# david-cortes/recometrics

Hardware: AMD Instinct MI355X
Metric: users/sec evaluated (all metrics, K=10) (higher is better)
Workload: dtype f32

## Files before the change

### recometrics_amd/csrc/rm_lib.hip

```cpp
#include <hip/hip_runtime.h>

#include <algorithm>
#include <array>
#include <cmath>
#include <cstdio>
#include <cstring>
#include <cstdlib>
#include <type_traits>
#include <atomic>
#include <chrono>
#include <condition_variable>
#include <csignal>
#include <functional>
#include <limits>
#include <map>
#include <memory>
#include <mutex>
#include <string>
#include <thread>
#include <vector>

#include "../../include/recometrics_hip.h"
#include "rm_device.hpp"
#include "rm_prep.hpp"
#include "rm_launch.hpp"
#include "rm_finalize.hpp"
#include "rm_noise.hpp"
#include "rm_scores.hpp"
#include "rm_rowtopk.hpp"

namespace {

using namespace rm;

thread_local std::string g_err;
struct RmError { int code; std::string msg; };

#define HIP_CHECK(expr)                                                                                   \
    do {                                                                                                  \
        hipError_t e_ = (expr);                                                                           \
        if (e_ != hipSuccess)                                                                             \
            throw RmError{e_ == hipErrorOutOfMemory ? RM_ERR_NOMEM : RM_ERR_HIP,                          \
                          std::string(#expr) + ": " + hipGetErrorString(e_)};                             \
    } while (0)

struct Switches {
    bool no_train_bits, no_spec, no_side, ext_topk, no_test_mask, hbm_lists, nsub2, no_pending, no_pos_beside, no_seed, rank_generic,
         no_fused_auc, no_defer_auc, noise_sequential, one_context, noise_per_batch, host_trace, no_pos_flat, no_row_topk, no_split_cache;
    long long free_mb, stream_budget_mb, noise_budget_mb, lane_cap_min, lane_min_k, lane_cap_set, sample_seed, split_cache_mb;
    unsigned long long epoch = 0;
    double batch_users;
    std::string splits;
    static bool on(const char *name) { return getenv(name) != nullptr; }
    static long long num(const char *name) { const char *e = getenv(name); return e ? atoll(e) : -1; }
    void load()
    {
        no_train_bits = on("RM_DEBUG_NO_TRAIN_BITS"); no_spec = on("RM_DEBUG_NO_SPEC"); no_side = on("RM_DEBUG_NO_SIDE");
        ext_topk = on("RM_DEBUG_EXT_TOPK"); no_test_mask = on("RM_DEBUG_NO_TEST_MASK");
        hbm_lists = on("RM_DEBUG_HBM_LISTS"); nsub2 = on("RM_DEBUG_NSUB2"); no_pending = on("RM_DEBUG_NO_PENDING");
        no_pos_beside = on("RM_DEBUG_NO_POS_BESIDE"); no_seed = on("RM_DEBUG_NO_SEED");
        rank_generic = on("RM_DEBUG_RANK_GENERIC"); no_fused_auc = on("RM_DEBUG_NO_FUSED_AUC");
        no_defer_auc = on("RM_DEBUG_NO_DEFER_AUC"); noise_sequential = on("RM_DEBUG_NOISE_SEQUENTIAL");
        one_context = on("RM_DEBUG_ONE_CONTEXT"); noise_per_batch = on("RM_DEBUG_NOISE_PER_BATCH"); host_trace = on("RM_HOST_TRACE");
        no_pos_flat = on("RM_DEBUG_NO_POS_FLAT");
        no_row_topk = on("RM_DEBUG_NO_ROW_TOPK");
        free_mb = num("RM_DEBUG_FREE_MB"); stream_budget_mb = num("RM_STREAM_BUDGET_MB");
        noise_budget_mb = num("RM_NOISE_BUDGET_MB");
        lane_min_k = num("RM_DEBUG_LANE_MIN_K");
        lane_cap_set = num("RM_DEBUG_LANE_CAP");
        sample_seed = num("RM_DEBUG_SAMPLE_SEED");
        lane_cap_min = num("RM_DEBUG_LANE_CAP_MIN");
        no_split_cache = on("RM_DEBUG_NO_SPLIT_CACHE");
        split_cache_mb = num("RM_SPLIT_CACHE_MB");
        epoch++;
        const char *b = getenv("RM_BATCH_USERS"); batch_users = b ? atof(b) : 0.0;
        const char *s = getenv("RM_DEBUG_SPLITS"); splits = s ? s : "";
    }
    Switches() { load(); }
};
Switches g_sw;

std::atomic<long long> g_ws_bytes{0};
inline long long debug_free_cap()
{
    return g_sw.free_mb >= 0 ? (g_sw.free_mb << 20) : -1;
}

struct RunTrace {
    std::mutex mu; std::vector<std::pair<const char *, double>> pts; std::chrono::steady_clock::time_point t0 = std::chrono::steady_clock::now();
    void point(const char *what) { std::lock_guard<std::mutex> lk(mu); if (pts.size() > 4096) pts.clear(); pts.emplace_back(what, std::chrono::duration<double, std::milli>(std::chrono::steady_clock::now() - t0).count()); }
};
RunTrace g_run_trace;
#define RM_TRACE_POINT(what) do { if (g_sw.host_trace) g_run_trace.point(what); } while (0)

std::atomic<unsigned long long> g_ws_stamp{1};
// ... 52 lines not shown
constexpr long long SPLIT_CACHE_DEFAULT_MB = 1024;
struct SplitKey {
    const void *arr[SPLIT_ARRAYS]; long long words[SPLIT_ARRAYS], nnz_train, nnz_test;
    int m, n, k, K, elem, req, min_items_pool, min_pos_test, heavy_npos, ng;
    int cold, cumulative, want_lane, ext_topk, allow_stream, force_stream, dense_ok, flat_early, csr_checked, rank_out;
    unsigned long long switches;
};
struct SplitCache {
    static constexpr const char *copy_names[SPLIT_ARRAYS] = {"split_train_p", "split_train_i", "split_test_p", "split_test_i", "split_test_v"};
    bool valid = false; SplitKey key{}; Plan hp{}; bool check_nan = false, dense_masked = false;
    std::vector<std::pair<std::string, unsigned long long>> stamps;
    void invalidate() { valid = false; }
    void keep(const Workspace &ws, const char *name) { stamps.emplace_back(name, ws.peek(name).stamp); }
    bool holds(const Workspace &ws, const SplitKey &k) const
    {
        if (!valid || std::memcmp(&key, &k, sizeof(SplitKey)) != 0) return false;
        for (const auto &s : stamps) if (s.second == 0 || ws.peek(s.first.c_str()).stamp != s.second) return false;
        return true;
    }
    const void *copy(const Workspace &ws, int i) const { return ws.peek(copy_names[i]).ptr; }
};
enum SideMark { SIDE_FORK, SIDE_JOIN, SIDE_PLAN_FORK, SIDE_CHECKS_DONE, SIDE_ROWS_AND_PACKS, SIDE_ROWS_FOR_POS, SIDE_TOP_VALUES,
                SIDE_SWEEP_FORK, SIDE_SWEEP_DEEP_DONE, SIDE_MERGED, SIDE_VERDICT, SIDE_SPLIT_KEPT, SIDE_MARKS };
enum PosMark { POS_PLAN_FORK, POS_MAXIMA_DONE, POS_SCORES_AFTER_COPY, POS_SCORES_DONE, POS_TABLES_INIT, POS_STREAMED_PLACED, POS_MARKS };
enum PassEvent { EV_START, EV_PREP_END , EV_SWEEP_END, EV_END, EV_COUNT };
struct NoiseWords {
    int first_early;
    int first_final;
    int sequential;
    int range_early;
    int batch_flagged;
};
static_assert(sizeof(NoiseWords) <= 64, "the noise words share one 64-byte page-locked allocation");
struct Ctx {
    int device = 0, slot = 0;
    std::mutex mu;
    Workspace ws;
    hipEvent_t ev[EV_COUNT] = {nullptr, nullptr, nullptr, nullptr};
    bool ev_valid = false, ev_recorded = false;
    hipStream_t side_stream = nullptr; std::array<hipEvent_t, SIDE_MARKS> side_marks{};
    hipStream_t pos_stream = nullptr; std::array<hipEvent_t, POS_MARKS> pos_marks{};
    hipEvent_t done = nullptr;
    hipStream_t own_stream = nullptr;
    hipStream_t up_stream = nullptr;
    hipEvent_t up_ev[2] = {nullptr, nullptr};
    NoiseWords *noise_words = nullptr; hipEvent_t flags_ev = nullptr, pass_ev = nullptr;
    void need_noise_words()
    {
        if (noise_words) return;
        HIP_CHECK(hipHostMalloc((void **)&noise_words, 64, hipHostMallocDefault));
        HIP_CHECK(hipEventCreateWithFlags(&flags_ev, hipEventDisableTiming));
        HIP_CHECK(hipEventCreateWithFlags(&pass_ev, hipEventDisableTiming));
    }
    void *pinned = nullptr; size_t pinned_bytes = 0;
    void *pinned_get(size_t bytes)
    {
        if (pinned_bytes < bytes) {
            if (pinned) { (void)hipHostFree(pinned); pinned = nullptr; pinned_bytes = 0; }
            if (hipHostMalloc(&pinned, bytes + bytes / 8, hipHostMallocDefault) != hipSuccess) { pinned = nullptr; throw RmError{RM_ERR_NOMEM, "hipHostMalloc of the output staging buffer failed"}; }
            pinned_bytes = bytes + bytes / 8;
        }
        return pinned;
    }
    double timings[8] = {0, 0, 0, 0, 0, 0, 0, 0};
// ... 326 lines not shown
inline void launch_csr_checks(int m, int n, const int *train_p, const int *train_i, long long nnz_train, const int *test_p, const int *test_i, long long nnz_test,
                              Plan *plan, const unsigned char *, hipStream_t stream)
{
    hipLaunchKernelGGL(k_check_csr_ptr, dim3(cdiv(m, 256)), dim3(256), 0, stream, m, train_p, nnz_train, test_p, nnz_test, plan);
    launch_csr_index_checks(m, n, train_p, train_i, nnz_train, test_p, test_i, nnz_test, plan, stream);
}
template <class T>
void check_csr_now(const Call<T> &c, hipStream_t stream, Ctx &cx)
{
    Plan *plan = (Plan *)cx.ws.get("plan", sizeof(Plan));
    cx.split.invalidate();
    if (cx.ev_valid) HIP_CHECK(hipStreamWaitEvent(stream, cx.done, 0));
    HIP_CHECK(hipMemsetAsync(plan, 0, sizeof(Plan), stream));
    launch_csr_checks(c.m, c.n, c.train_p, c.train_i, c.nnz_train, c.test_p, c.test_i, c.nnz_test, plan, c.only_users, stream);
    Plan hp;
    HIP_CHECK(hipMemcpyAsync(&hp, plan, sizeof(Plan), hipMemcpyDeviceToHost, stream));
    HIP_CHECK(hipStreamSynchronize(stream));
    throw_csr_defects(hp, c, cx);
}

struct Beside {
    hipStream_t &st; hipEvent_t *const ev; const int n_ev; const hipStream_t call; const bool high_priority; bool enabled;
    long long handed = 0, joined = 0, at[SIDE_MARKS] = {};
    static_assert((int)POS_MARKS <= (int)SIDE_MARKS, "at[] holds the roles of either stream");
    Beside(hipStream_t &s, hipEvent_t *e, int n, hipStream_t call_, bool hp, bool on_) : st(s), ev(e), n_ev(n), call(call_), high_priority(hp), enabled(on_) {}
    ~Beside() { if (handed > joined && st) (void)hipStreamSynchronize(st); }
    hipStream_t get()
    {
        if (!st) {
            HIP_CHECK(create_stream(&st, high_priority));
            for (int i = 0; i < n_ev; i++) HIP_CHECK(hipEventCreateWithFlags(&ev[i], hipEventDisableTiming));
        }
        return st;
    }
    hipStream_t on() { if (!enabled) return call; handed++; return get(); }
    void cut(int role) { if (enabled) { get(); HIP_CHECK(hipEventRecord(ev[role], call)); } }
    hipStream_t behind(int role) { if (!enabled) return call; HIP_CHECK(hipStreamWaitEvent(st, ev[role], 0)); handed++; return st; }
    hipStream_t fork(int role) { cut(role); return behind(role); }
    void mark(int role) { if (enabled) { HIP_CHECK(hipEventRecord(ev[role], st)); at[role] = handed; } }
    void joined_at(int role) { joined = std::max(joined, at[role]); at[role] = 0; }
    void await(int role, hipStream_t into) { if (enabled) { HIP_CHECK(hipStreamWaitEvent(into, ev[role], 0)); if (into == call) joined_at(role); } }
    void join(int role) { mark(role); await(role, call); }
    bool marked(int role) const { return at[role] != 0; }
    void sync() { if (enabled && st) { HIP_CHECK(hipStreamSynchronize(st)); joined = handed; } }
    void host_wait(int role) { if (enabled) { HIP_CHECK(hipEventSynchronize(ev[role])); joined_at(role); } }
};

// ... 88 lines not shown

inline Geometry scores_geometry(const Plan &hp, int n, bool want_auc)
{
    Geometry g{};
    g.jmax = want_auc ? hp.jmax : 0;
    g.n_ublocks = (hp.n_groups + GROUPS_PER_BLOCK - 1) / GROUPS_PER_BLOCK;
    g.nsub = 2; g.tile_items = TILE_ITEMS; g.n_waves = 8;
    g.tiles_total = (n + TILE_ITEMS - 1) / TILE_ITEMS;
    g.n_splits = 1; g.part_splits = 1; g.n_part = 1;
    g.u_split = 0; g.j_shallow = -1;
    return g;
}

template <class T>
struct Pipeline {
    typedef Prec<T> P;
    typedef typename std::remove_pointer<decltype(typename P::Args{}.thr_shared)>::type ThrT;
    static constexpr int GU = P::GU;
    Call<T> c;
    hipStream_t stream; Ctx &cx; Workspace &ws;
    const int m, n, k, K;
    const bool use_side = !g_sw.no_side;
    Beside side, pos;
    int min_items_pool = 0, min_pos_test = 0, req = 0, NG = 0; bool want_auc = false;
    int *flags = nullptr, *user_nslots = nullptr, *uslot_base = nullptr, *heavy_users = nullptr; Plan *plan = nullptr;
    int *slot_user = nullptr, *slot_chunk = nullptr, *slot_index = nullptr, *gj = nullptr, *sc_user = nullptr, *sc_chunk = nullptr;
    long long *grow = nullptr; double *log2tab = nullptr;
    ClassifyArgs ca{};
    bool want_lane = false, ext_topk = false, items_known = false, dense_ok = false;
    bool row_topk = false;
    bool bits_early = false, bits_early_masked = false, masked_from_bits = false, flat_early = false;
    bool allow_reuse = true, reused = false, keepable = false; SplitKey split_key{};
    Plan hp{};
    int n_slots = 0, n_stream = 0, stream_slot0 = 0; bool check_nan = false;
    Geometry g{};
    FinalArgs<T, T> fa{};
    Entry<T> *merged = nullptr; long long *rank_sorted = nullptr;
    T *pos_score = nullptr; unsigned *hist = nullptr; int *pos_order = nullptr, *pos_item = nullptr;
    Entry<T> *pl = nullptr; PartialStat<T> *pst = nullptr;
    T *stream_scores = nullptr, *spos_score = nullptr; int *spos_item = nullptr; unsigned *shist = nullptr;
    long long stream_ld = 0;
    typename P::Args sa{};
    typename P::ListT *glists = nullptr; int *lane_cnt = nullptr; ThrT *thr_shared = nullptr;
    bool lane_lists = false;
    bool collect = false; CollectGeom collect_g{};

    Pipeline(const Call<T> &c_, hipStream_t s, Ctx &cx_)
        : c(c_), stream(s), cx(cx_), ws(cx_.ws), m(c_.m), n(c_.n), k(c_.k), K(c_.K),
          side(cx_.side_stream, cx_.side_marks.data(), SIDE_MARKS, s, cx_.high_priority, use_side),
          pos(cx_.pos_stream, cx_.pos_marks.data(), POS_MARKS, s, cx_.high_priority, use_side) {}

    void begin()
    {
        min_items_pool = std::max(std::max(c.min_items_pool, K), 2);
        min_pos_test = std::min(c.min_pos_test, 1);
        if (c.reco) { min_items_pool = 1; min_pos_test = 0; }
        for (int i = 0; i < 10; i++) if (c.out[i] && !c.reco) req |= (1 << i);
        want_auc = req & (RQ_ROC | RQ_PR);
        NG = c.scores ? 2 : P::supported_ng(k);
        if (NG < 0) throw RmError{RM_ERR_UNSUPPORTED, std::string(P::limit()) + " (got " + std::to_string(k) + ")"};
        if (!cx.ev_valid) {
            for (int i = 0; i < EV_COUNT; i++) HIP_CHECK(hipEventCreate(&cx.ev[i]));
            HIP_CHECK(hipEventCreateWithFlags(&cx.done, hipEventDisableTiming));
            cx.ev_valid = true;
        } else {
            HIP_CHECK(hipStreamWaitEvent(stream, cx.done, 0));
        }
        g_last_ctx = &cx;
        HIP_CHECK(hipEventRecord(cx.ev[EV_START], stream));
        RM_TRACE_POINT("run: start");
    }

    void plan_stage()
// ... 97 lines not shown
            side.mark(SIDE_CHECKS_DONE);
            if (!c.scores) hipLaunchKernelGGL(k_absmax<T>, dim3(512), dim3(256), 0, aux2, c.A, c.lda, (long long)m, k, &plan->amax_a, &plan->nonfinite);
            if (!items_known && !c.scores) hipLaunchKernelGGL(k_absmax<T>, dim3(1024), dim3(256), 0, aux2, c.B, c.ldb, (long long)n, k, &plan->amax_b, &plan->nonfinite_b);
            pos.mark(POS_MAXIMA_DONE);
            if (attempt == 0 && flat_early) hipLaunchKernelGGL(k_entry_users, dim3(cdiv(cdiv(m, WAVE) * WAVE, 256)), dim3(256), 0, pos.on(), m, c.test_p, ent_user, plan);
            if (attempt == 0 && std::is_same<T, float>::value && use_side && !c.ext_bits && dense_ok) {
                SweepArgs probe{};
                const bool guess = want_auc && !ext_topk && !g_sw.no_test_mask;
                (void)ws.get("train_bits", (size_t)m * (size_t)dense_row_words(n) * 4);
                if (!(c.same_train_rows && cx.dense.fits(ws, m, dense_row_words(n), guess))) {
                    set_train_bits(probe, cx, c, m, n, dense_ok, side.on(), guess, false, false, flat_early ? ent_masked : nullptr);
                    side.mark(SIDE_ROWS_AND_PACKS); side.mark(SIDE_ROWS_FOR_POS);
                    bits_early = true; bits_early_masked = guess; masked_from_bits = flat_early;
                }
            }
            side.await(SIDE_CHECKS_DONE, stream); pos.await(POS_MAXIMA_DONE, stream);
            HIP_CHECK(hipMemcpyAsync(cx.pinned_plan, plan, sizeof(Plan), hipMemcpyDeviceToHost, stream));
            if (attempt == 0 && flat_early) {
                const hipStream_t sc = pos.fork(POS_SCORES_AFTER_COPY);
                if (c.scores) {
                    hipLaunchKernelGGL(k_test_masked, dim3(cdiv(m, TM_USERS)), dim3(256), 0, sc, m, c.test_p, c.test_i, c.train_p, c.train_i, ent_user, ent_masked, plan);
                    hipLaunchKernelGGL(k_pos_scores_given<T>, dim3(cdiv(c.nnz_test, 256)), dim3(256), 0, sc, pf, c.S, c.lds, (const int *)ent_user, (const unsigned char *)ent_masked);
                } else {
                hipLaunchKernelGGL(k_pos_scores_flat<T>, dim3(cdiv(c.nnz_test, POSF_WAVES * WAVE)), dim3(POSF_WAVES * WAVE), 0, sc, pf, ent_user);
                if (masked_from_bits) side.await(SIDE_ROWS_FOR_POS, sc);
                else hipLaunchKernelGGL(k_test_masked, dim3(cdiv(m, TM_USERS)), dim3(256), 0, sc, m, c.test_p, c.test_i, c.train_p, c.train_i, ent_user, ent_masked, plan);
                hipLaunchKernelGGL(k_pos_apply_masked<T>, dim3(cdiv(c.nnz_test, 256)), dim3(256), 0, sc, pf, ent_masked);
                }
                pos.mark(POS_SCORES_DONE);
            }
            RM_TRACE_POINT("run: plan chain + side kernels enqueued");
            HIP_CHECK(hipStreamSynchronize(stream));
            RM_TRACE_POINT("run: plan read back");
            hp = *cx.pinned_plan;
            throw_csr_defects(hp, c, cx);
            if (ca.allow_stream && !ca.force_stream && hp.class_count[STREAM_CLASS] > stream_cap && attempt == 0) {
                ca.allow_stream = 0; ca.check_ptr = 0; keepable = false;
                side.sync(); pos.sync();
                continue;
            }
            break;
        }
        if (!reused) throw_csr_defects(hp, c, cx);
        n_slots = hp.n_slots;
        n_stream = (want_auc || ext_topk) ? hp.class_count[STREAM_CLASS] : 0;
        stream_slot0 = n_stream > 0 ? hp.class_offset[STREAM_CLASS] : n_slots;
        if (!reused) check_nan = scores_may_overflow();
// ... 12 lines not shown
    bool make_split_key(SplitKey &key) const
    {
        std::memset(&key, 0, sizeof(SplitKey));
        if (g_sw.no_split_cache || !use_side || c.reco || c.scores || c.noise || c.only_users || c.ext_bits || c.noise_E || c.noise_flag ||
            c.first_pass_flags || c.flag_snapshot || c.items_tag != 0 || !c.test_p || m <= 0) return false;
        const void *arr[SPLIT_ARRAYS] = {c.train_p, c.train_i, c.test_p, c.test_i, c.test_v};
        const long long words[SPLIT_ARRAYS] = {(long long)m + 1, std::max<long long>(c.nnz_train, 0), (long long)m + 1, std::max<long long>(c.nnz_test, 0),
                                               c.test_v ? std::max<long long>(c.nnz_test, 0) * (long long)(sizeof(T) / 4) : 0};
        long long total = 0;
        for (int i = 0; i < SPLIT_ARRAYS; i++) { key.arr[i] = arr[i]; key.words[i] = words[i]; total += words[i]; }
        if (total * 4 > ((g_sw.split_cache_mb >= 0 ? g_sw.split_cache_mb : SPLIT_CACHE_DEFAULT_MB) << 20)) return false;
        key.nnz_train = c.nnz_train; key.nnz_test = c.nnz_test;
        key.m = m; key.n = n; key.k = k; key.K = K; key.elem = (int)sizeof(T); key.req = req;
        key.min_items_pool = min_items_pool; key.min_pos_test = min_pos_test; key.heavy_npos = ca.heavy_npos; key.ng = NG;
        key.cold = c.cold; key.cumulative = c.cumulative; key.want_lane = want_lane; key.ext_topk = ext_topk;
        key.allow_stream = ca.allow_stream; key.force_stream = ca.force_stream; key.dense_ok = dense_ok; key.flat_early = flat_early;
        key.csr_checked = c.csr_checked; key.rank_out = (c.topk_idx ? 1 : 0) | (c.pos_rank ? 2 : 0) | (c.status ? 4 : 0);
        key.switches = g_sw.epoch;
        return true;
    }
    void plan_reused(const PosArgs<T> &pf, const int *ent_user, const unsigned char *ent_masked, const void *const theirs[SPLIT_ARRAYS])
    {
        const SplitCache &kept = cx.split;
        const size_t at = offsetof(Plan, split_differs);
        HIP_CHECK(hipMemsetAsync((char *)plan + at, 0, offsetof(Plan, csr_bad) - at, stream));
        const hipStream_t aux = side.fork(SIDE_PLAN_FORK);
        SplitSameArgs ss{};
        long long longest = 1;
        for (int i = 0; i < SPLIT_ARRAYS; i++) {
            ss.theirs[i] = (const unsigned *)theirs[i]; ss.ours[i] = (const unsigned *)kept.copy(ws, i); ss.words[i] = kept.key.words[i];
            longest = std::max(longest, ss.words[i]);
        }
        ss.plan = plan;
        const unsigned blocks = (unsigned)std::min<long long>(SPLIT_SAME_BLOCKS, cdiv(cdiv(longest, 4), SPLIT_SAME_THREADS));
        hipLaunchKernelGGL(k_split_same, dim3(blocks), dim3(SPLIT_SAME_THREADS), 0, aux, ss);
        hipLaunchKernelGGL(k_absmax<T>, dim3(512), dim3(256), 0, aux, c.A, c.lda, (long long)m, k, &plan->amax_a, &plan->nonfinite);
        hipLaunchKernelGGL(k_absmax<T>, dim3(1024), dim3(256), 0, aux, c.B, c.ldb, (long long)n, k, &plan->amax_b, &plan->nonfinite_b);
        HIP_CHECK(hipMemcpyAsync(cx.pinned_plan, plan, sizeof(Plan), hipMemcpyDeviceToHost, aux));
        side.mark(SIDE_VERDICT);
        if (flat_early) {
            const hipStream_t sc = pos.fork(POS_PLAN_FORK);
            hipLaunchKernelGGL(k_pos_scores_flat<T>, dim3(cdiv(c.nnz_test, POSF_WAVES * WAVE)), dim3(POSF_WAVES * WAVE), 0, sc, pf, ent_user);
            hipLaunchKernelGGL(k_pos_apply_masked<T>, dim3(cdiv(c.nnz_test, 256)), dim3(256), 0, sc, pf, ent_masked);
            pos.mark(POS_SCORES_DONE);
        }
        check_launch(hipGetLastError());
        hp = kept.hp; check_nan = kept.check_nan;
        bits_early = dense_ok; bits_early_masked = kept.dense_masked; masked_from_bits = true;
        RM_TRACE_POINT("run: kept split, comparison + positives enqueued");
    }
    bool verdict()
    {
        side.host_wait(SIDE_VERDICT);
        RM_TRACE_POINT("run: verdict read back");
        const Plan &rb = *cx.pinned_plan;
        hp.amax_a = rb.amax_a; hp.amax_b = rb.amax_b; hp.nonfinite = rb.nonfinite; hp.nonfinite_b = rb.nonfinite_b;
        if (!rb.split_differs && scores_may_overflow() == check_nan) { cx.split_reused = 1; return true; }
        side.sync(); pos.sync();
        HIP_CHECK(hipStreamSynchronize(stream));
        cx.split.invalidate(); cx.dense.invalidate(); cx.packed.invalidate();
        cx.split_reused = 0;
        return false;
    }
    void keep_split()
    {
        if (!keepable || reused) return;
        SplitCache &kept = cx.split;
        void *dst[SPLIT_ARRAYS] = {};
        try { for (int i = 0; i < SPLIT_ARRAYS; i++) if (split_key.words[i] > 0) dst[i] = ws.get(SplitCache::copy_names[i], (size_t)split_key.words[i] * 4); }
        catch (const RmError &) { keepable = false; return; }
        const hipStream_t st = side.on();
        for (int i = 0; i < SPLIT_ARRAYS; i++)
            if (dst[i]) HIP_CHECK(hipMemcpyAsync(dst[i], split_key.arr[i], (size_t)split_key.words[i] * 4, hipMemcpyDeviceToDevice, st));
        side.mark(SIDE_SPLIT_KEPT);
        std::memcpy(&kept.key, &split_key, sizeof(SplitKey));
        kept.hp = hp; kept.check_nan = check_nan; kept.dense_masked = dense_ok && cx.dense.masked;
        kept.stamps.clear();
        for (const char *name : {"flags", "user_nslots", "uslot_base", "plan", "heavy_users", "slot_user", "slot_chunk", "slot_index", "slot_j", "gj", "grow", "sc_user", "sc_chunk"})
            kept.keep(ws, name);
        if (flat_early) { kept.keep(ws, "ent_user"); kept.keep(ws, "ent_masked"); }
        if (dense_ok) kept.keep(ws, "train_bits");
// ... 55 lines not shown
        if (bits_early && (bits_early_masked != g.mask_test || (g.use_ext_bits && dense_ok))) side.await(SIDE_ROWS_AND_PACKS, stream);
        if (g.use_ext_bits && dense_ok) set_ext_bits(sa, c.ext_bits, (int)c.ext_words);
        else set_train_bits(sa, cx, c, m, n, dense_ok, stream, g.mask_test, bits_early, bits_early_masked);

        if (want_auc) positives();

        if (n_stream > 0) stream_scores = (T *)ws.get("stream_scores", sizeof(T) * (size_t)n_stream * (size_t)stream_ld);
        if (!ext_topk) pl = (Entry<T> *)ws.get("pl", sizeof(Entry<T>) * (size_t)n_slots * g.n_part * K);
        pst = (PartialStat<T> *)ws.get("pst", sizeof(PartialStat<T>) * (size_t)n_slots * g.n_part);
        const unsigned n_blocks = (unsigned)((g.n_ublocks - g.tail_ublocks) * g.n_splits + g.tail_ublocks * g.tail_splits);
        lane_lists = want_lane && !ext_topk;
        int lane_cap = lane_lists ? P::lane_cap(K) : 0;
        if (lane_lists && g_sw.lane_cap_set > 0) lane_cap = (int)std::min<long long>(std::max<long long>(P::lane_cap(K), (g_sw.lane_cap_set + 15) / 16 * 16), (COLLECT_MAX_ENTRIES - K) / 16 * 16);
        if (lane_lists && g_sw.lane_cap_min >= 0)
            lane_cap = std::min(lane_cap, (K + lane_sel_slack(K) + 16 + 1 + 15) / 16 * 16);
        if (lane_lists) {
            glists = (typename P::ListT *)ws.get("glists", (size_t)n_blocks * g.n_waves * WAVE * (size_t)lane_cap * (sizeof(T) + 4));
            lane_cnt = (int *)ws.get("lane_cnt", sizeof(int) * (size_t)n_blocks * g.n_waves * WAVE);
        } else if (!g.list_in_lds && !ext_topk) {
            glists = (typename P::ListT *)ws.get("glists", sizeof(typename P::ListT) * (size_t)n_blocks * g.n_waves * GU * (2 * K + 32));
        }

        thr_shared = (ThrT *)ws.get("thr_shared", sizeof(ThrT) * (size_t)n_slots);
        if (want_auc && !ext_topk && !g_sw.no_seed)
            hipLaunchKernelGGL((k_seed_thresholds<T, ThrT>), dim3(cdiv(n_slots, 256)), dim3(256), 0, stream, n_slots, stream_slot0, K, GU, slot_user, slot_chunk,
                               user_nslots, flags, c.test_p, grow, pos_score, spos_score, thr_shared);
        else HIP_CHECK(hipMemsetAsync(thr_shared, 0, sizeof(ThrT) * (size_t)n_slots, stream));
        sa.thr_shared = thr_shared;
        sa.n = n; sa.K = K; sa.ngt = NG; sa.n_slots = n_slots; sa.n_groups = n_groups; sa.n_ublocks = g.n_ublocks;
        sa.n_splits = g.n_splits; sa.tail_ublocks = g.tail_ublocks; sa.tail_splits = g.tail_splits; sa.part_splits = g.part_splits; sa.tiles_total = tiles_total; sa.jmax = g.jmax; sa.check_nan = check_nan ? 1 : 0; sa.buffered_lists = (want_lane || ext_topk) ? 1 : 0; sa.ext_topk = ext_topk ? 1 : 0;
        sa.Ap = (decltype(sa.Ap))Ap; sa.Bp = (decltype(sa.Bp))Bp; sa.slot_user = slot_user; sa.slot_chunk = slot_chunk;
        sa.train_p = c.train_p; sa.train_i = c.train_i; sa.gj = gj; sa.grow = grow;
        sa.pos_score = pos_score; sa.pos_item = pos_item; sa.hist = hist; sa.glists = glists; sa.lane_cap = lane_cap; sa.lane_cnt = lane_cnt; sa.pl = pl; sa.pst = pst; sa.dump = nullptr;
        P::set_pending(sa, g.pend_cap, 0);
        P::set_sync(sa, (int)g.sync_off);
        sa.stream_slot0 = stream_slot0; sa.stream_ld = stream_ld; sa.stream_scores = stream_scores;
        set_part_extra(sa, g.part_extra);
        sa.noise_row = c.noise_row; sa.noise_row0 = c.noise_row0; sa.noise_E = c.noise_E; sa.noise_ld = c.noise_ld;
        set_spec(sa);

        if (side.marked(SIDE_ROWS_AND_PACKS)) side.await(SIDE_ROWS_AND_PACKS, stream);
        const bool sample_lists = !lane_lists && !ext_topk && sizeof(T) == 4;
        const int sample_S = (lane_lists || sample_lists) ? sample_seed_items<T>(ws, K, n, n_slots, check_nan || c.noise_E != nullptr, sample_lists) : 0;
        if (sample_S > 0 && !sample_lists) seed_from_sample<T>(sa, ws, sample_S, NG, n_slots, g.n_ublocks, stream);
        else if (sample_S > 0) {
            const long long units = P::items_units(sample_S / TILE_ITEMS, NG);
            typename P::PackT *Bs = (typename P::PackT *)ws.get("sample_items", 16 * (size_t)units);
            void *Ls = ws.get("sample_lists", sizeof(typename P::ListT) * (size_t)g.n_ublocks * 8 * GU * (2 + 32));
            pack_operands(c.A, c.lda, c.B, c.ldb, sample_S, k, NG, TILE_ITEMS, slot_user, 0, Ap, 0, Bs, units, stream, true);
            seed_from_sample<T>(sa, ws, sample_S, NG, n_slots, g.n_ublocks, stream, Bs, Ls);
        }
        RM_TRACE_POINT("run: preparation enqueued");
    }

    void positives()
    {
        const int n_groups = hp.n_groups;
        const long long rows = hp.total_rows + n_groups;
        pos_score = (T *)ws.get("pos_score", sizeof(T) * (size_t)(rows + 1) * GU);
        pos_item = (int *)ws.get("pos_item", sizeof(int) * (size_t)(rows + 1) * GU);
        hist = (unsigned *)ws.get("hist", sizeof(unsigned) * (size_t)(rows + 1) * GU);
        T *pos_tmp = (T *)ws.get("pos_tmp", sizeof(T) * (size_t)std::max<long long>(c.nnz_test, 1));
        pos_order = (int *)ws.get("pos_order", sizeof(int) * (size_t)std::max<long long>(c.nnz_test, 1));
        PosArgs<T> pa{m, n, k, c.A, c.lda, c.B, c.ldb, c.train_p, c.train_i, c.test_p, c.test_i,
                      flags, user_nslots, uslot_base, slot_index, grow, pos_tmp, pos_order, pos_score, pos_item, GU};
        pa.noise_row = c.noise_row; pa.noise_row0 = c.noise_row0; pa.noise_E = c.noise_E; pa.noise_ld = c.noise_ld;
        pa.noise_flag = c.noise_flag; pa.plan = plan;
        if (sizeof(T) == 4)
            pa.pos_key = (unsigned long long *)ws.get("pos_key", 8 * ((size_t)std::max<long long>(c.nnz_test, 1) + 8));
        const bool flat = flat_early;
        const bool pos_beside = use_side && n_stream > 0 && stream_slot0 > 0 && !g_sw.no_pos_beside;
        hipStream_t ps = pos_beside ? pos.on() : stream;
        PosArgs<T> pb = pa;
        const hipStream_t fill = (flat && pos_beside) ? stream : ps;
        if (n_stream > 0) {
            const size_t nz = (size_t)std::max<long long>(c.nnz_test, 1);
            spos_score = (T *)ws.get("spos_score", sizeof(T) * nz);
            spos_item = (int *)ws.get("spos_item", sizeof(int) * nz);
            shist = (unsigned *)ws.get("shist", sizeof(unsigned) * nz);
            pb.stream = 1; pb.spos_score = spos_score; pb.spos_item = spos_item;
            hipLaunchKernelGGL(k_init_tables<T>, dim3(cdiv((long long)nz, 256)), dim3(256), 0, fill, spos_score, shist, (long long)nz);
        }
        const int nsc = hp.n_stream_chunks;
        hipLaunchKernelGGL(k_init_tables<T>, dim3(cdiv(rows * GU, 256)), dim3(256), 0, stream, pos_score, hist, rows * GU);
        if (flat) {
            if (pos_beside) ps = pos.fork(POS_TABLES_INIT);
            pos.await(POS_SCORES_DONE, stream);
        } else {
            if (n_stream > 0) hipLaunchKernelGGL(k_pos_scores<T>, dim3(cdiv(nsc, POSS_WAVES)), dim3(POSS_WAVES * WAVE), 0, ps, pb, sc_user, sc_chunk, nsc);
            if (stream_slot0 > 0) hipLaunchKernelGGL(k_pos_scores<T>, dim3(cdiv(stream_slot0, POSS_WAVES)), dim3(POSS_WAVES * WAVE), 0, stream, pa, slot_user, slot_chunk, stream_slot0);
        }
        if (n_stream > 0) hipLaunchKernelGGL(k_pos_place<T>, dim3(cdiv((long long)nsc * WAVE, 256)), dim3(256), 0, ps, pb, sc_user, sc_chunk, nsc);
        if (stream_slot0 > 0) hipLaunchKernelGGL(k_pos_place<T>, dim3(cdiv((long long)stream_slot0 * WAVE, 256)), dim3(256), 0, stream, pa, slot_user, slot_chunk, stream_slot0);
        if (pos_beside) pos.join(POS_STREAMED_PLACED);
    }

    void sweep()
    {
        if (c.flag_snapshot) {
            if (n_slots > 0) {
                HIP_CHECK(hipMemcpyAsync(c.flag_snapshot, c.noise_flag, sizeof(int) * (size_t)m, hipMemcpyDeviceToDevice, stream));
                HIP_CHECK(hipMemcpyAsync(c.flag_count_host, &plan->n_noise_flagged, sizeof(int), hipMemcpyDeviceToHost, stream));
            } else {
                HIP_CHECK(hipMemsetAsync(c.flag_snapshot, 0, sizeof(int) * (size_t)m, stream));
                *c.flag_count_host = 0;
            }
            HIP_CHECK(hipEventRecord(c.flags_event, stream));
        }
        HIP_CHECK(hipEventRecord(cx.ev[EV_PREP_END], stream));
        double *tm = cx.timings;
        if (n_slots == 0) {
            HIP_CHECK(hipEventRecord(cx.ev[EV_SWEEP_END], stream));
            tm[4] = 0; tm[5] = 0; tm[6] = 0; tm[7] = 0;
            return;
        }
// ... 1431 lines not shown
```

### recometrics_amd/csrc/rm_prep.hpp

```cpp
#pragma once
#include "rm_device.hpp"

namespace rm {

struct ClassifyArgs {
    int m, n, K;
    const int *train_p, *test_p;
    int req;
    int cold, min_items_pool, min_pos_test;
    int want_auc;
    int *flags;
    int *user_nslots;
    int *heavy_users;
    Plan *plan;
    const unsigned char *only;
    int force_stream;
    int allow_stream;
    int check_ptr;
    int heavy_npos;
    long long nnz_train, nnz_test;
    int reco;
};

__device__ __forceinline__ int chunk_depth(int pc)
// ... 397 lines not shown
__device__ __forceinline__ KeyT seed_of_slot(int slot, int stream_slot0, int K, int gu, const int *slot_user, const int *slot_chunk, const int *user_nslots,
                                             const int *flags, const int *test_p, const long long *grow, const T *pos_score, const T *spos_score)
{
    const int u = slot_user[slot];
    if (slot_chunk[slot] != 0 || user_nslots[u] != 1 || (flags[u] & UF_ONLY_NDCG)) return (KeyT)0;
    const int te0 = test_p[u], P = test_p[u + 1] - te0;
    if (P < K) return (KeyT)0;
    const T *tab; long long stride;
    if (slot >= stream_slot0) { tab = spos_score + te0; stride = 1; }
    else { const int g = slot / gu; tab = pos_score + (grow[g] + g) * gu + (slot % gu); stride = gu; }
    int nvalid = P;
    while (nvalid > 0) { const T x = tab[(long long)(nvalid - 1) * stride]; if (isinf(x) && x > 0) nvalid--; else break; }
    if (nvalid < K) return (KeyT)0;
    int i = nvalid - 1, distinct = 1;
    T kth = tab[(long long)i * stride];
    while (distinct < K && i > 0) {
        const T x = tab[(long long)(--i) * stride];
        if (x != kth && !(isinf(x) && x > 0)) { kth = x; distinct++; }
    }
    if (distinct < K) return (KeyT)0;
    return kth == kth ? (KeyT)ord_key(kth) : (KeyT)0;
}
template <class T, class KeyT>
__global__ void k_seed_thresholds(int n_slots, int stream_slot0, int K, int gu, const int *slot_user, const int *slot_chunk, const int *user_nslots,
                                  const int *flags, const int *test_p, const long long *grow, const T *pos_score, const T *spos_score, KeyT *thr_shared)
{
    const int slot = blockIdx.x * blockDim.x + threadIdx.x;
    if (slot >= n_slots) return;
    thr_shared[slot] = seed_of_slot<T, KeyT>(slot, stream_slot0, K, gu, slot_user, slot_chunk, user_nslots, flags, test_p, grow, pos_score, spos_score);
}

template <class S, class KeyT, int NV>
__global__ __launch_bounds__(256) void k_seed_from_sample(int n_slots, int K, const S *sample, const int *slot_user, const int *slot_chunk,
                                                          const int *train_p, const int *train_i, KeyT *thr_shared)
{
    constexpr int SN = NV * WAVE;
    __shared__ unsigned masked[4][SN / 32];
    const int wv = threadIdx.x >> 6, lane = threadIdx.x & 63;
    const int slot = blockIdx.x * 4 + wv;
    if (slot >= n_slots || slot_chunk[slot] != 0) return;
    const int u = slot_user[slot];
    if (u < 0) return;
    KeyT key[NV];
    const S *row = sample + (size_t)slot * SN;
    #pragma unroll
    for (int j = 0; j < NV; j++) { const S x = row[j * WAVE + lane]; key[j] = x == x ? (KeyT)ord_key(x) : (KeyT)0; }
    for (int w = lane; w < SN / 32; w += WAVE) masked[wv][w] = 0u;
    __builtin_amdgcn_fence(__ATOMIC_ACQ_REL, "wavefront"); __builtin_amdgcn_wave_barrier();
    const int tr0 = train_p[u], tr1 = train_p[u + 1];
    for (int i0 = tr0; i0 < tr1; i0 += WAVE) {
// ... 259 lines not shown
        }
    }
    for (; t < k; t++) s = __builtin_fma(x[t], y[t], s);
    return s;
}

template <class T> struct PosArgs {
    int m, n, k;
    const T *A; size_t lda; const T *B; size_t ldb;
    const int *train_p, *train_i, *test_p, *test_i;
    const int *flags, *user_nslots, *uslot_base, *slot_index;
    const long long *grow;
    T *pos_tmp;
    int *pos_order;
    T *pos_score;
    int *pos_item;
    int gu;
    const int *noise_row; int noise_row0; const T *noise_E; long long noise_ld;
    int *noise_flag; Plan *plan;
    int stream;
    T *spos_score;
    int *spos_item;
    unsigned long long *pos_key;
};

__device__ __forceinline__ bool in_sorted_row(const int *row, int len, int item)
{
    int lo = 0, hi = len;
    while (lo < hi) { const int mid = (lo + hi) >> 1; if (row[mid] < item) lo = mid + 1; else hi = mid; }
    return lo < len && row[lo] == item;
}

__device__ __forceinline__ float fma_chain_step(float a, float b, float s) { return __builtin_fmaf(a, b, s); }
__device__ __forceinline__ double fma_chain_step(double a, double b, double s) { return __builtin_fma(a, b, s); }

constexpr int POSS_WAVES = 4;
template <class T>
__global__ __launch_bounds__(POSS_WAVES * WAVE) void k_pos_scores(PosArgs<T> a, const int *slot_user, const int *slot_chunk, int n_slots)
{
    constexpr int PB = 128;
    constexpr int CH = PB / (int)sizeof(T);
    constexpr int VE = 16 / (int)sizeof(T);
    constexpr int LPR = PB / 16;
    constexpr int RPI = WAVE / LPR;
    constexpr int LD = CH + VE;
    typedef T VT __attribute__((ext_vector_type(16 / sizeof(T))));
// ... 116 lines not shown
                        lo[q] = lt ? mid + 1 : lo[q];
                        n[q] = lt ? n[q] - half - 1 : half;
                    }
                }
                #pragma unroll
                for (int q = 0; q < EB; q++) { const int e = e0 + q * 256; if (e < e_end) ent_masked[e] = lo[q] < end[q] && seg[lo[q]] == item[q]; }
            } else {
                #pragma unroll
                for (int q = 0; q < EB; q++) {
                    const int e = e0 + q * 256;
                    if (e >= e_end) continue;
                    const int tr0 = trp[ul[q]], ntr = trp[ul[q] + 1] - tr0;
                    ent_masked[e] = ntr && in_sorted_row(train_i + tr0, ntr, item[q]);
                }
            }
        }
        __syncthreads();
        a = b;
    }
}

constexpr int POSF_WAVES = 4;
template <class T>
__global__ __launch_bounds__(POSF_WAVES * WAVE) void k_pos_scores_flat(PosArgs<T> a, const int *ent_user)
{
    constexpr int PB = 64;
    constexpr int CH = PB / (int)sizeof(T);
    constexpr int VE = 16 / (int)sizeof(T);
    constexpr int LPR = PB / 16;
    constexpr int RPI = WAVE / LPR;
    constexpr int LD = CH + VE;
    typedef T VT __attribute__((ext_vector_type(16 / sizeof(T))));
    __shared__ __attribute__((aligned(16))) T rows[POSF_WAVES][WAVE][LD];
    if (a.plan->csr_bad & (CSR_BAD_INDPTR | CSR_BAD_INDEX)) return;
    const int wv = __builtin_amdgcn_readfirstlane(threadIdx.x >> 6), lane = threadIdx.x & 63;
    const long long e = (long long)a.test_p[0] + ((long long)blockIdx.x * POSF_WAVES + wv) * WAVE + lane;
    const bool in = e < (long long)a.test_p[a.m];
    const int u = in ? ent_user[e] : 0;
    const int item = in ? a.test_i[e] : 0;
    const int f = in ? a.flags[u] : 0;
    const bool mine = in && (f & UF_ACTIVE) && !(f & UF_ONLY_NDCG);
    const unsigned long long live = __ballot(mine);
    if (!live) return;
    const int rsub = lane / LPR, piece = lane % LPR;
    const bool vec_ok = ((((size_t)a.B) | (a.ldb * sizeof(T))) & 15) == 0, avec_ok = ((((size_t)a.A) | (a.lda * sizeof(T))) & 15) == 0;
    const T *brow[WAVE / RPI];
    #pragma unroll
    for (int q = 0; q < WAVE / RPI; q++) brow[q] = a.B + (size_t)__shfl(item, q * RPI + rsub) * a.ldb;
    const T *Au = a.A + (size_t)u * a.lda;
    T s = 0;
    for (int k0 = 0; k0 < a.k; k0 += CH) {
        const int e0 = k0 + piece * VE;
        VT bv[WAVE / RPI];
        #pragma unroll
        for (int q = 0; q < WAVE / RPI; q++) {
            const int p = q * RPI + rsub;
            VT x;
            #pragma unroll
            for (int i = 0; i < VE; i++) x[i] = (T)0;
            if (((live >> p) & 1) && e0 < a.k) {
                if (vec_ok && e0 + VE <= a.k) x = *(const VT *)(brow[q] + e0);
                else {
                    #pragma unroll
// ... 27 lines not shown
            for (int j = 0; j < CH / VE; j++) {
                const VT b = *(const VT *)(r + j * VE);
                #pragma unroll
                for (int i = 0; i < VE; i++) s = fma_chain_step(av[j][i], b[i], s);
            }
        } else {
            #pragma unroll
            for (int j = 0; j < CH / VE; j++) {
                const VT b = *(const VT *)(r + j * VE);
                #pragma unroll
                for (int i = 0; i < VE; i++) if (k0 + j * VE + i < a.k) s = fma_chain_step(av[j][i], b[i], s);
            }
        }
        __builtin_amdgcn_fence(__ATOMIC_ACQ_REL, "wavefront"); __builtin_amdgcn_wave_barrier();
    }
    if (mine && a.noise_E) {
        const long long nr = a.noise_row ? a.noise_row[u] - a.noise_row0 : u;
        s += a.noise_E[(size_t)nr * (size_t)a.noise_ld + item];
    }
    if (mine && a.noise_flag && (s < (T)0 ? -s : s) < (T)6.103515625e-05f) {
        if (atomicExch(&a.noise_flag[u], 1) == 0) atomicAdd(&a.plan->n_noise_flagged, 1);
    }
    if (mine) {
        a.pos_tmp[e] = s;
        if (sizeof(T) == 4 && a.pos_key) a.pos_key[e] = ((unsigned long long)ord_key((float)s) << 32) | (unsigned)~item;
    }
}
template <class T>
__global__ void k_pos_apply_masked(PosArgs<T> a, const unsigned char *ent_masked)
{
    if (a.plan->csr_bad & (CSR_BAD_INDPTR | CSR_BAD_INDEX)) return;
    const long long e = (long long)a.test_p[0] + (long long)blockIdx.x * blockDim.x + threadIdx.x;
    if (e >= (long long)a.test_p[a.m] || !ent_masked[e]) return;
    const T inf = (T)__int_as_float(0x7f800000);
    a.pos_tmp[e] = inf;
    if (sizeof(T) == 4 && a.pos_key) a.pos_key[e] = ((unsigned long long)ord_key((float)inf) << 32) | (unsigned)~a.test_i[e];
}

constexpr int PLACE_THREADS = 256;
template <class T>
__global__ __launch_bounds__(PLACE_THREADS) void k_pos_place(PosArgs<T> a, const int *slot_user, const int *slot_chunk, int n_slots)
{
    const int w = __builtin_amdgcn_readfirstlane((blockIdx.x * blockDim.x + threadIdx.x) >> 6), lane = threadIdx.x & 63;
    if (w >= n_slots) return;
    const int u = slot_user[w], c0 = slot_chunk[w];
    if (a.flags[u] & UF_ONLY_NDCG) return;
    const int te0 = a.test_p[u], te1 = a.test_p[u + 1];
    const int e = te0 + c0 * POS_CHUNK + lane;
    const bool mine = lane < POS_CHUNK && e < te1;
    const T s = mine ? a.pos_tmp[e] : (T)0;
    const int item = mine ? a.test_i[e] : 0;
    int rank = 0;
    if (sizeof(T) == 4 && a.pos_key) {
        __shared__ __attribute__((aligned(16))) unsigned long long kbuf[PLACE_THREADS / WAVE][2][WAVE];
        const int wv = __builtin_amdgcn_readfirstlane(threadIdx.x >> 6);
        const unsigned long long key = ((unsigned long long)ord_key((float)s) << 32) | (unsigned)~item;
        const unsigned long long *keys = a.pos_key + te0;
        const int P = te1 - te0;
        unsigned long long nxt = lane < P ? keys[lane] : ~0ull;
        for (int j0 = 0; j0 < P; j0 += WAVE) {
            const unsigned long long cur = nxt;
            if (j0 + WAVE < P) nxt = j0 + WAVE + lane < P ? keys[j0 + WAVE + lane] : ~0ull;
            unsigned long long *kb = kbuf[wv][(j0 >> 6) & 1];
            kb[lane] = cur;
            __builtin_amdgcn_fence(__ATOMIC_ACQ_REL, "wavefront");
            __builtin_amdgcn_wave_barrier();
            const int cnt = min(WAVE, P - j0);
            typedef unsigned long long K2 __attribute__((ext_vector_type(2)));
            for (int j = 0; j < cnt; j += 16) {
// ... 6 lines not shown
        for (int f0 = te0; f0 < te1; f0 += WAVE) {
            const int f = f0 + lane;
            const unsigned kh = f < te1 ? ord_key((float)a.pos_tmp[f]) : 0u;
            const unsigned kl = f < te1 ? (unsigned)~a.test_i[f] : 0u;
            const int cnt = min(WAVE, te1 - f0);
            for (int j = 0; j < cnt; j++) {
                const unsigned long long kj = ((unsigned long long)(unsigned)lane_bcast<int>((int)kh, j) << 32) | (unsigned)lane_bcast<int>((int)kl, j);
                rank += kj < key;
            }
        }
    } else {
        for (int f0 = te0; f0 < te1; f0 += WAVE) {
            const int f = f0 + lane;
            const T sf = f < te1 ? a.pos_tmp[f] : (T)0;
            const int itf = f < te1 ? a.test_i[f] : 0;
            const int cnt = min(WAVE, te1 - f0);
            for (int j = 0; j < cnt; j++) {
                const T sj = lane_bcast<T>(sf, j);
                const int ij = lane_bcast<int>(itf, j);
                rank += (sj < s) || (sj == s && ij > item);
            }
        }
    }
    if (mine && a.stream) {
        a.pos_order[e] = rank;
        a.spos_score[te0 + rank] = s;
        a.spos_item[te0 + rank] = item;
    } else if (mine) {
        a.pos_order[e] = rank;
        const int c = rank / POS_CHUNK, r = rank % POS_CHUNK;
        const int slot = a.slot_index[a.uslot_base[u] + c];
        const long long at = (a.grow[slot / a.gu] + slot / a.gu + r) * a.gu + (slot % a.gu);
        a.pos_score[at] = s;
        a.pos_item[at] = item;
    }
}

}
```

Measured before the change: 18.19 million.

## Fuse masking into flat positive scoring and compute threshold seeds during placement

On the reused-split path, masking is folded into k_pos_scores_flat, so masked entries get +inf directly and the separate k_pos_apply_masked launch is dropped. The positive-score launch is issued before the verification work, which moves to a new high-priority urgent stream and waits for the scores. Threshold seeds for non-streamed slots are now computed inside k_pos_place from the in-wave sorted row instead of a separate k_seed_thresholds pass, with streamed slots seeded right after placement. This cuts kernel launches and a pass over the data, at the cost of an extra stream, cross-stream dependencies, and more complex seed logic inside the placement kernel.

After: 18.16 million. About the same (-0.2%).

```diff
diff --git a/recometrics_amd/csrc/rm_lib.hip b/recometrics_amd/csrc/rm_lib.hip
--- a/recometrics_amd/csrc/rm_lib.hip
+++ b/recometrics_amd/csrc/rm_lib.hip
@@ -46,7 +46,7 @@
 
 struct Switches {
     bool no_train_bits, no_spec, no_side, ext_topk, no_test_mask, hbm_lists, nsub2, no_pending, no_pos_beside, no_seed, rank_generic,
-         no_fused_auc, no_defer_auc, noise_sequential, one_context, noise_per_batch, host_trace, no_pos_flat, no_row_topk, no_split_cache;
+         no_fused_auc, no_defer_auc, noise_sequential, one_context, noise_per_batch, host_trace, no_pos_flat, no_row_topk, no_split_cache, no_prep_fusion;
     long long free_mb, stream_budget_mb, noise_budget_mb, lane_cap_min, lane_min_k, lane_cap_set, sample_seed, split_cache_mb;
     unsigned long long epoch = 0;
     double batch_users;
@@ -71,6 +71,7 @@
         sample_seed = num("RM_DEBUG_SAMPLE_SEED");
         lane_cap_min = num("RM_DEBUG_LANE_CAP_MIN");
         no_split_cache = on("RM_DEBUG_NO_SPLIT_CACHE");
+        no_prep_fusion = on("RM_DEBUG_NO_PREP_FUSION");
         split_cache_mb = num("RM_SPLIT_CACHE_MB");
         epoch++;
         const char *b = getenv("RM_BATCH_USERS"); batch_users = b ? atof(b) : 0.0;
@@ -169,6 +170,7 @@
 };
 enum SideMark { SIDE_FORK, SIDE_JOIN, SIDE_PLAN_FORK, SIDE_CHECKS_DONE, SIDE_ROWS_AND_PACKS, SIDE_ROWS_FOR_POS, SIDE_TOP_VALUES,
                 SIDE_SWEEP_FORK, SIDE_SWEEP_DEEP_DONE, SIDE_MERGED, SIDE_VERDICT, SIDE_SPLIT_KEPT, SIDE_MARKS };
+enum UrgentMark { URGENT_PLAN_FORK, URGENT_VERDICT, URGENT_MARKS };
 enum PosMark { POS_PLAN_FORK, POS_MAXIMA_DONE, POS_SCORES_AFTER_COPY, POS_SCORES_DONE, POS_TABLES_INIT, POS_STREAMED_PLACED, POS_MARKS };
 enum PassEvent { EV_START, EV_PREP_END , EV_SWEEP_END, EV_END, EV_COUNT };
 struct NoiseWords {
@@ -187,6 +189,7 @@
     bool ev_valid = false, ev_recorded = false;
     hipStream_t side_stream = nullptr; std::array<hipEvent_t, SIDE_MARKS> side_marks{};
     hipStream_t pos_stream = nullptr; std::array<hipEvent_t, POS_MARKS> pos_marks{};
+    hipStream_t urgent_stream = nullptr; std::array<hipEvent_t, URGENT_MARKS> urgent_marks{};
     hipEvent_t done = nullptr;
     hipStream_t own_stream = nullptr;
     hipStream_t up_stream = nullptr;
@@ -559,7 +562,7 @@
 struct Beside {
     hipStream_t &st; hipEvent_t *const ev; const int n_ev; const hipStream_t call; const bool high_priority; bool enabled;
     long long handed = 0, joined = 0, at[SIDE_MARKS] = {};
-    static_assert((int)POS_MARKS <= (int)SIDE_MARKS, "at[] holds the roles of either stream");
+    static_assert((int)POS_MARKS <= (int)SIDE_MARKS && (int)URGENT_MARKS <= (int)SIDE_MARKS, "at[] holds the roles of every stream");
     Beside(hipStream_t &s, hipEvent_t *e, int n, hipStream_t call_, bool hp, bool on_) : st(s), ev(e), n_ev(n), call(call_), high_priority(hp), enabled(on_) {}
     ~Beside() { if (handed > joined && st) (void)hipStreamSynchronize(st); }
     hipStream_t get()
@@ -694,6 +697,7 @@
     const int m, n, k, K;
     const bool use_side = !g_sw.no_side;
     Beside side, pos;
+    Beside urgent;
     int min_items_pool = 0, min_pos_test = 0, req = 0, NG = 0; bool want_auc = false;
     int *flags = nullptr, *user_nslots = nullptr, *uslot_base = nullptr, *heavy_users = nullptr; Plan *plan = nullptr;
     int *slot_user = nullptr, *slot_chunk = nullptr, *slot_index = nullptr, *gj = nullptr, *sc_user = nullptr, *sc_chunk = nullptr;
@@ -703,6 +707,7 @@
     bool row_topk = false;
     bool bits_early = false, bits_early_masked = false, masked_from_bits = false, flat_early = false;
     bool allow_reuse = true, reused = false, keepable = false; SplitKey split_key{};
+    bool fused = false;
     Plan hp{};
     int n_slots = 0, n_stream = 0, stream_slot0 = 0; bool check_nan = false;
     Geometry g{};
@@ -720,7 +725,8 @@
     Pipeline(const Call<T> &c_, hipStream_t s, Ctx &cx_)
         : c(c_), stream(s), cx(cx_), ws(cx_.ws), m(c_.m), n(c_.n), k(c_.k), K(c_.K),
           side(cx_.side_stream, cx_.side_marks.data(), SIDE_MARKS, s, cx_.high_priority, use_side),
-          pos(cx_.pos_stream, cx_.pos_marks.data(), POS_MARKS, s, cx_.high_priority, use_side) {}
+          pos(cx_.pos_stream, cx_.pos_marks.data(), POS_MARKS, s, cx_.high_priority, use_side),
+          urgent(cx_.urgent_stream, cx_.urgent_marks.data(), URGENT_MARKS, s, true, use_side) {}
 
     void begin()
     {
@@ -864,7 +870,7 @@
                     hipLaunchKernelGGL(k_test_masked, dim3(cdiv(m, TM_USERS)), dim3(256), 0, sc, m, c.test_p, c.test_i, c.train_p, c.train_i, ent_user, ent_masked, plan);
                     hipLaunchKernelGGL(k_pos_scores_given<T>, dim3(cdiv(c.nnz_test, 256)), dim3(256), 0, sc, pf, c.S, c.lds, (const int *)ent_user, (const unsigned char *)ent_masked);
                 } else {
-                hipLaunchKernelGGL(k_pos_scores_flat<T>, dim3(cdiv(c.nnz_test, POSF_WAVES * WAVE)), dim3(POSF_WAVES * WAVE), 0, sc, pf, ent_user);
+                hipLaunchKernelGGL(k_pos_scores_flat<T>, dim3(cdiv(c.nnz_test, POSF_WAVES * WAVE)), dim3(POSF_WAVES * WAVE), 0, sc, pf, ent_user, (const unsigned char *)nullptr);
                 if (masked_from_bits) side.await(SIDE_ROWS_FOR_POS, sc);
                 else hipLaunchKernelGGL(k_test_masked, dim3(cdiv(m, TM_USERS)), dim3(256), 0, sc, m, c.test_p, c.test_i, c.train_p, c.train_i, ent_user, ent_masked, plan);
                 hipLaunchKernelGGL(k_pos_apply_masked<T>, dim3(cdiv(c.nnz_test, 256)), dim3(256), 0, sc, pf, ent_masked);
@@ -923,9 +929,19 @@
     void plan_reused(const PosArgs<T> &pf, const int *ent_user, const unsigned char *ent_masked, const void *const theirs[SPLIT_ARRAYS])
     {
         const SplitCache &kept = cx.split;
+        fused = !g_sw.no_prep_fusion;
+        auto scores = [&]() {
+            if (!flat_early) return;
+            const hipStream_t sc = pos.fork(POS_PLAN_FORK);
+            hipLaunchKernelGGL(k_pos_scores_flat<T>, dim3(cdiv(c.nnz_test, POSF_WAVES * WAVE)), dim3(POSF_WAVES * WAVE), 0, sc, pf, ent_user, fused ? ent_masked : (const unsigned char *)nullptr);
+            if (!fused) hipLaunchKernelGGL(k_pos_apply_masked<T>, dim3(cdiv(c.nnz_test, 256)), dim3(256), 0, sc, pf, ent_masked);
+            pos.mark(POS_SCORES_DONE);
+        };
+        if (fused) scores();
         const size_t at = offsetof(Plan, split_differs);
         HIP_CHECK(hipMemsetAsync((char *)plan + at, 0, offsetof(Plan, csr_bad) - at, stream));
-        const hipStream_t aux = side.fork(SIDE_PLAN_FORK);
+        hipStream_t aux = side.fork(SIDE_PLAN_FORK);
+        if (fused) aux = urgent.fork(URGENT_PLAN_FORK);
         SplitSameArgs ss{};
         long long longest = 1;
         for (int i = 0; i < SPLIT_ARRAYS; i++) {
@@ -934,17 +950,16 @@
         }
         ss.plan = plan;
         const unsigned blocks = (unsigned)std::min<long long>(SPLIT_SAME_BLOCKS, cdiv(cdiv(longest, 4), SPLIT_SAME_THREADS));
-        hipLaunchKernelGGL(k_split_same, dim3(blocks), dim3(SPLIT_SAME_THREADS), 0, aux, ss);
+        if (!fused) hipLaunchKernelGGL(k_split_same, dim3(blocks), dim3(SPLIT_SAME_THREADS), 0, aux, ss);
         hipLaunchKernelGGL(k_absmax<T>, dim3(512), dim3(256), 0, aux, c.A, c.lda, (long long)m, k, &plan->amax_a, &plan->nonfinite);
         hipLaunchKernelGGL(k_absmax<T>, dim3(1024), dim3(256), 0, aux, c.B, c.ldb, (long long)n, k, &plan->amax_b, &plan->nonfinite_b);
+        if (fused) {
+            if (flat_early) pos.await(POS_SCORES_DONE, aux);
+            hipLaunchKernelGGL(k_split_same, dim3(blocks), dim3(SPLIT_SAME_THREADS), 0, aux, ss);
+        }
         HIP_CHECK(hipMemcpyAsync(cx.pinned_plan, plan, sizeof(Plan), hipMemcpyDeviceToHost, aux));
-        side.mark(SIDE_VERDICT);
-        if (flat_early) {
-            const hipStream_t sc = pos.fork(POS_PLAN_FORK);
-            hipLaunchKernelGGL(k_pos_scores_flat<T>, dim3(cdiv(c.nnz_test, POSF_WAVES * WAVE)), dim3(POSF_WAVES * WAVE), 0, sc, pf, ent_user);
-            hipLaunchKernelGGL(k_pos_apply_masked<T>, dim3(cdiv(c.nnz_test, 256)), dim3(256), 0, sc, pf, ent_masked);
-            pos.mark(POS_SCORES_DONE);
-        }
+        if (fused) urgent.mark(URGENT_VERDICT); else side.mark(SIDE_VERDICT);
+        if (!fused) scores();
         check_launch(hipGetLastError());
         hp = kept.hp; check_nan = kept.check_nan;
         bits_early = dense_ok; bits_early_masked = kept.dense_masked; masked_from_bits = true;
@@ -952,12 +967,12 @@
     }
     bool verdict()
     {
-        side.host_wait(SIDE_VERDICT);
+        if (fused) urgent.host_wait(URGENT_VERDICT); else side.host_wait(SIDE_VERDICT);
         RM_TRACE_POINT("run: verdict read back");
         const Plan &rb = *cx.pinned_plan;
         hp.amax_a = rb.amax_a; hp.amax_b = rb.amax_b; hp.nonfinite = rb.nonfinite; hp.nonfinite_b = rb.nonfinite_b;
         if (!rb.split_differs && scores_may_overflow() == check_nan) { cx.split_reused = 1; return true; }
-        side.sync(); pos.sync();
+        side.sync(); pos.sync(); urgent.sync();
         HIP_CHECK(hipStreamSynchronize(stream));
         cx.split.invalidate(); cx.dense.invalidate(); cx.packed.invalidate();
         cx.split_reused = 0;
@@ -1059,8 +1074,9 @@
         }
 
         thr_shared = (ThrT *)ws.get("thr_shared", sizeof(ThrT) * (size_t)n_slots);
-        if (want_auc && !ext_topk && !g_sw.no_seed)
-            hipLaunchKernelGGL((k_seed_thresholds<T, ThrT>), dim3(cdiv(n_slots, 256)), dim3(256), 0, stream, n_slots, stream_slot0, K, GU, slot_user, slot_chunk,
+        if (seeds_in_place()) ;
+        else if (want_auc && !ext_topk && !g_sw.no_seed)
+            hipLaunchKernelGGL((k_seed_thresholds<T, ThrT>), dim3(cdiv(n_slots, 256)), dim3(256), 0, stream, 0, n_slots, stream_slot0, K, GU, slot_user, slot_chunk,
                                user_nslots, flags, c.test_p, grow, pos_score, spos_score, thr_shared);
         else HIP_CHECK(hipMemsetAsync(thr_shared, 0, sizeof(ThrT) * (size_t)n_slots, stream));
         sa.thr_shared = thr_shared;
@@ -1089,6 +1105,8 @@
         }
         RM_TRACE_POINT("run: preparation enqueued");
     }
+
+    bool seeds_in_place() const { return fused && want_auc && !ext_topk && !g_sw.no_seed; }
 
     void positives()
     {
@@ -1119,6 +1137,10 @@
             hipLaunchKernelGGL(k_init_tables<T>, dim3(cdiv((long long)nz, 256)), dim3(256), 0, fill, spos_score, shist, (long long)nz);
         }
         const int nsc = hp.n_stream_chunks;
+        if (seeds_in_place()) {
+            thr_shared = (ThrT *)ws.get("thr_shared", sizeof(ThrT) * (size_t)n_slots);
+            pa.thr_seed = thr_shared; pa.seed_K = K;
+        }
         hipLaunchKernelGGL(k_init_tables<T>, dim3(cdiv(rows * GU, 256)), dim3(256), 0, stream, pos_score, hist, rows * GU);
         if (flat) {
             if (pos_beside) ps = pos.fork(POS_TABLES_INIT);
@@ -1128,6 +1150,9 @@
             if (stream_slot0 > 0) hipLaunchKernelGGL(k_pos_scores<T>, dim3(cdiv(stream_slot0, POSS_WAVES)), dim3(POSS_WAVES * WAVE), 0, stream, pa, slot_user, slot_chunk, stream_slot0);
         }
         if (n_stream > 0) hipLaunchKernelGGL(k_pos_place<T>, dim3(cdiv((long long)nsc * WAVE, 256)), dim3(256), 0, ps, pb, sc_user, sc_chunk, nsc);
+        if (n_stream > 0 && seeds_in_place())
+            hipLaunchKernelGGL((k_seed_thresholds<T, ThrT>), dim3(cdiv(n_slots - stream_slot0, 256)), dim3(256), 0, ps, stream_slot0, n_slots, stream_slot0, K, GU, slot_user, slot_chunk,
+                               user_nslots, flags, c.test_p, grow, pos_score, spos_score, thr_shared);
         if (stream_slot0 > 0) hipLaunchKernelGGL(k_pos_place<T>, dim3(cdiv((long long)stream_slot0 * WAVE, 256)), dim3(256), 0, stream, pa, slot_user, slot_chunk, stream_slot0);
         if (pos_beside) pos.join(POS_STREAMED_PLACED);
     }
diff --git a/recometrics_amd/csrc/rm_prep.hpp b/recometrics_amd/csrc/rm_prep.hpp
--- a/recometrics_amd/csrc/rm_prep.hpp
+++ b/recometrics_amd/csrc/rm_prep.hpp
@@ -443,10 +443,10 @@
     return kth == kth ? (KeyT)ord_key(kth) : (KeyT)0;
 }
 template <class T, class KeyT>
-__global__ void k_seed_thresholds(int n_slots, int stream_slot0, int K, int gu, const int *slot_user, const int *slot_chunk, const int *user_nslots,
+__global__ void k_seed_thresholds(int slot0, int n_slots, int stream_slot0, int K, int gu, const int *slot_user, const int *slot_chunk, const int *user_nslots,
                                   const int *flags, const int *test_p, const long long *grow, const T *pos_score, const T *spos_score, KeyT *thr_shared)
 {
-    const int slot = blockIdx.x * blockDim.x + threadIdx.x;
+    const int slot = slot0 + blockIdx.x * blockDim.x + threadIdx.x;
     if (slot >= n_slots) return;
     thr_shared[slot] = seed_of_slot<T, KeyT>(slot, stream_slot0, K, gu, slot_user, slot_chunk, user_nslots, flags, test_p, grow, pos_score, spos_score);
 }
@@ -752,6 +752,7 @@
     T *spos_score;
     int *spos_item;
     unsigned long long *pos_key;
+    void *thr_seed; int seed_K;
 };
 
 __device__ __forceinline__ bool in_sorted_row(const int *row, int len, int item)
@@ -914,7 +915,7 @@
 
 constexpr int POSF_WAVES = 4;
 template <class T>
-__global__ __launch_bounds__(POSF_WAVES * WAVE) void k_pos_scores_flat(PosArgs<T> a, const int *ent_user)
+__global__ __launch_bounds__(POSF_WAVES * WAVE) void k_pos_scores_flat(PosArgs<T> a, const int *ent_user, const unsigned char *ent_masked)
 {
     constexpr int PB = 64;
     constexpr int CH = PB / (int)sizeof(T);
@@ -931,6 +932,7 @@
     const int u = in ? ent_user[e] : 0;
     const int item = in ? a.test_i[e] : 0;
     const int f = in ? a.flags[u] : 0;
+    const bool masked = in && ent_masked && ent_masked[e];
     const bool mine = in && (f & UF_ACTIVE) && !(f & UF_ONLY_NDCG);
     const unsigned long long live = __ballot(mine);
     if (!live) return;
@@ -1004,8 +1006,9 @@
         if (atomicExch(&a.noise_flag[u], 1) == 0) atomicAdd(&a.plan->n_noise_flagged, 1);
     }
     if (mine) {
-        a.pos_tmp[e] = s;
-        if (sizeof(T) == 4 && a.pos_key) a.pos_key[e] = ((unsigned long long)ord_key((float)s) << 32) | (unsigned)~item;
+        const T sv = masked ? (T)__int_as_float(0x7f800000) : s;
+        a.pos_tmp[e] = sv;
+        if (sizeof(T) == 4 && a.pos_key) a.pos_key[e] = ((unsigned long long)ord_key((float)sv) << 32) | (unsigned)~item;
     }
 }
 template <class T>
@@ -1026,7 +1029,9 @@
     const int w = __builtin_amdgcn_readfirstlane((blockIdx.x * blockDim.x + threadIdx.x) >> 6), lane = threadIdx.x & 63;
     if (w >= n_slots) return;
     const int u = slot_user[w], c0 = slot_chunk[w];
-    if (a.flags[u] & UF_ONLY_NDCG) return;
+    typedef decltype(ord_key(T())) SeedT;
+    SeedT *const seed = a.stream ? nullptr : (SeedT *)a.thr_seed;
+    if (a.flags[u] & UF_ONLY_NDCG) { if (seed && lane == 0) seed[w] = (SeedT)0; return; }
     const int te0 = a.test_p[u], te1 = a.test_p[u + 1];
     const int e = te0 + c0 * POS_CHUNK + lane;
     const bool mine = lane < POS_CHUNK && e < te1;
@@ -1079,6 +1084,34 @@
             }
         }
     }
+    if (seed) {
+        __shared__ T seed_row[PLACE_THREADS / WAVE][WAVE];
+        const int P = te1 - te0, K = a.seed_K;
+        SeedT out = (SeedT)0;
+        bool writer = lane == 0;
+        if (c0 == 0 && a.user_nslots[u] == 1 && P >= K && P <= POS_CHUNK) {
+            T *row = seed_row[__builtin_amdgcn_readfirstlane(threadIdx.x >> 6)];
+            row[lane] = (T)__int_as_float(0x7f800000);
+            __builtin_amdgcn_fence(__ATOMIC_ACQ_REL, "wavefront"); __builtin_amdgcn_wave_barrier();
+            if (mine) row[rank] = s;
+            __builtin_amdgcn_fence(__ATOMIC_ACQ_REL, "wavefront"); __builtin_amdgcn_wave_barrier();
+            const T x = row[lane];
+            const bool pinf = isinf(x) && x > 0;
+            const unsigned long long finite = __ballot(lane < P && !pinf);
+            const int nvalid = finite ? 64 - __clzll((long long)finite) : 0;
+            if (nvalid >= K) {
+                const unsigned long long above = lane < WAVE - 1 ? finite & (~0ull << (lane + 1)) : 0ull;
+                const T y = __shfl(x, above ? __ffsll((long long)above) - 1 : lane);
+                const bool head = lane < P && !pinf && (!above || x != y);
+                const unsigned long long heads = __ballot(head);
+                if (__popcll(heads) >= K) {
+                    writer = head && __popcll(heads >> lane) == K;
+                    out = x == x ? (SeedT)ord_key(x) : (SeedT)0;
+                }
+            }
+        }
+        if (writer) seed[w] = out;
+    }
     if (mine && a.stream) {
         a.pos_order[e] = rank;
         a.spos_score[te0 + rank] = s;
```
